# sikang/motion_primitive_library

Hardware: AMD Instinct MI355X
Metric: node-expansions/s (frontier x |U| pair evaluations per second) (higher is better)
Workload: dtype f64; 1 GPU; C4: 3D VoxelMapUtil 512^3, Control::ACC |U|=729 (9^3), 64k-node synthetic frontier; frontier=random, frontier_nodes=65536, frontier_nodes_per_gpu=65536, controls=729, dim=3, map_cells=134217728, device=AMD Radeon Graphics (gfx950:sramecc+:xnack-), compute_units=256, kernel=expand_lex_kernel

## Files before the change

### motion_primitive_library_amd/csrc/expand_lex_kernel.hip

```cpp
#include "mplx_internal.h"
#include "mplx_device_common.h"

namespace mplx {

using namespace dev;

constexpr int kLexWPB = 4;
constexpr int kLexBT = 64 * kLexWPB;
constexpr int kLexTabStride = 64;
constexpr int kLexUB8 = 8;

constexpr int kShUval = 0;
__host__ __device__ constexpr int lex_sh_tc(int TS) { return TS == 32 ? 768 : 384; }
__host__ __device__ constexpr int lex_sh_tt(int TS) { return lex_sh_tc(TS) + 64; }
__host__ __device__ constexpr int lex_ts(int ndp) { return ndp <= 8 ? 8 : (ndp <= 16 ? 16 : 32); }

__host__ __device__ constexpr int lex_fixed_bytes(int D, int K, int TS) {
  const int F = 4 * D + 2, KQ = K == 3 ? 4 : K;
  int w = (F * 8 + 15) & ~15;
  w += 128 + D * TS * 4 + D * TS * 4 * KQ + D * TS * 8 * (K - 1) + (K == 3 ? D * TS * 8 : 0) + D * TS + D * TS;
  w = (w + 15) & ~15;
  return (w + 128 + 7) & ~7;
}
__host__ __device__ constexpr int lex_tt_entries(int n_max) { return (n_max + 1) * (n_max + 2) / 2; }

template <int D, int K, int TS>
struct LexW {
  static constexpr int F = 4 * D + 2;
  static constexpr int KQ = K == 3 ? 4 : K;
  static constexpr int NODE = 0;
  static constexpr int MISC = (F * 8 + 15) & ~15;
  static constexpr int EFLAG = MISC + 128;
  static constexpr int EQ = EFLAG + D * TS * 4;
  static constexpr int EST = EQ + D * TS * 4 * KQ;
  static constexpr int UQ = EST + D * TS * 8 * (K - 1);
  static constexpr int VL = UQ + (K == 3 ? D * TS * 8 : 0);
  static constexpr int VLC = VL + D * TS;
  static constexpr int ROWMAP = (VLC + D * TS + 15) & ~15;
  static constexpr int HP = (ROWMAP + 128 + 7) & ~7;
  static_assert(HP == lex_fixed_bytes(D, K, TS), "LexLds sizes the workgroup's LDS from lex_fixed_bytes");
};
enum { LM_BASE = 0, LM_NODEQ = 4 };

struct LexLds {
  int tts, rowcap, o_wave0, w_drop, w_cell, w_box, wave_bytes, total;
  __host__ __device__ LexLds(int D, int K, int waves, int ndp, int nU, int n_max, int rmax, int boxcap) {
    tts = n_max + 1;
    rowcap = rmax * tts;
    o_wave0 = (lex_sh_tt(lex_ts(ndp)) + lex_tt_entries(n_max) * 8 + 15) & ~15;
    int w = lex_fixed_bytes(D, K, lex_ts(ndp));
    const int PN = (D == 3) ? ndp * ndp : ndp;
    w += PN * 8;
    w_drop = w;
    w += ((nU + 63) >> 6) * 8;
    w_cell = w;
    w += D * ndp * rowcap + 8;
    w = (w + 3) & ~3;
    w_box = w;
    w += boxcap * 4;
    wave_bytes = (w + 15) & ~15;
    total = o_wave0 + waves * wave_bytes;
  }
};

namespace {

template <typename T>
__device__ __forceinline__ void lex_st(T v, T *p) {
// ... 20 lines not shown
  x = op(x, __builtin_amdgcn_update_dpp(id, v, 0x111, 0xf, 0xf, false));
  x = op(x, __builtin_amdgcn_update_dpp(id, v, 0x112, 0xf, 0xf, false));
  x = op(x, __builtin_amdgcn_update_dpp(id, v, 0x113, 0xf, 0xf, false));
  x = op(x, __builtin_amdgcn_update_dpp(id, x, 0x114, 0xf, 0xe, false));
  x = op(x, __builtin_amdgcn_update_dpp(id, x, 0x118, 0xf, 0xc, false));
  return x;
}
__device__ __forceinline__ unsigned int row_reduce_or(unsigned int v) {
  int x = (int)v;
  x |= __builtin_amdgcn_update_dpp(0, (int)v, 0x111, 0xf, 0xf, false);
  x |= __builtin_amdgcn_update_dpp(0, (int)v, 0x112, 0xf, 0xf, false);
  x |= __builtin_amdgcn_update_dpp(0, (int)v, 0x113, 0xf, 0xf, false);
  x |= __builtin_amdgcn_update_dpp(0, x, 0x114, 0xf, 0xe, false);
  x |= __builtin_amdgcn_update_dpp(0, x, 0x118, 0xf, 0xc, false);
  return (unsigned int)x;
}

template <int K>
__device__ __forceinline__ void lex_fold_entry(uint64_t &h, const int *eq, int e) {
  if (K == 1) {
    fold(h, eq[e]);
  } else if (K == 2) {
    const int2 q = *(const int2 *)(eq + e * 2);
    fold(h, q.x);
    fold(h, q.y);
  } else {
    const int4 q = *(const int4 *)(eq + e * 4);
    fold(h, q.x);
    fold(h, q.y);
    fold(h, q.z);
  }
}

template <int D, int K, int TS>
__global__ __launch_bounds__(kLexBT) void expand_lex_kernel(const GridArgs A_kernarg) {
  extern __shared__ __align__(16) unsigned char smem[];
  typedef const GridArgs __attribute__((address_space(4))) *KernargPtr;
  KernargPtr Ak = (KernargPtr)__builtin_amdgcn_kernarg_segment_ptr();
  (void)A_kernarg;
#define A (*Ak)
  typedef LexW<D, K, TS> W;
  constexpr int F = W::F, KQ = W::KQ;
  constexpr int UB = (D == 3 && K == 3) ? 4 : kLexUB8;
  const int ndp = A.ndp, RM = A.rmax;
  const LexLds L(D, K, kLexWPB, ndp, A.nU, A.n_max, RM, A.boxcap);
  const int lane = threadIdx.x & 63;
  const int wv = __builtin_amdgcn_readfirstlane(threadIdx.x >> 6);
  const double *s_uval = (const double *)(smem + kShUval);
  constexpr int kShTc = lex_sh_tc(TS), kShTt = lex_sh_tt(TS);
  const unsigned char *s_tc = smem + kShTc;
  const double *s_tt = (const double *)(smem + kShTt);
  unsigned char *wb = smem + L.o_wave0 + wv * L.wave_bytes;
  double *s_node = (double *)(wb + W::NODE);
  int *s_misc = (int *)(wb + W::MISC);
  int *s_eflag = (int *)(wb + W::EFLAG);
  int *s_eq = (int *)(wb + W::EQ);
  double *s_est = (double *)(wb + W::EST);
  double *s_uq = (double *)(wb + W::UQ);
  unsigned char *s_vl = wb + W::VL;
  unsigned char *s_vlc = wb + W::VLC;
  unsigned short *s_rowmap = (unsigned short *)(wb + W::ROWMAP);
  uint64_t *s_drop = (uint64_t *)(wb + L.w_drop);
  uint64_t *s_hp = (uint64_t *)(wb + W::HP);
  unsigned char *s_cell = wb + L.w_cell;
  unsigned int *s_box = (unsigned int *)(wb + L.w_box);

  const int tts = L.tts, rowcap = L.rowcap;
  const int half = A.n_max + 2;
  const double T = A.dt;
  const int dims[3] = {A.dim0, A.dim1, A.dim2};
  const int nd[3] = {A.nd0, A.nd1, A.nd2};

  const int wave_id = (int)blockIdx.x * kLexWPB + wv;
  const int wave_stride = (int)gridDim.x * kLexWPB;
  const int NN = (int)A.n_nodes;
  const bool dyn = A.work != nullptr;
  const int ck = dyn ? A.work_chunk : 1;
  int dyn_beg = 0, dyn_len = 0, dyn_step = 1;
  unsigned int *ctr = nullptr;
  if (dyn) {
    if (blockIdx.x == 0 && threadIdx.x < kWorkCounters) A.work_zero[threadIdx.x * 32] = 0u;
    const int n_chunks = (NN + ck - 1) / ck, n_dyn = n_chunks > wave_stride ? n_chunks - wave_stride : 0;
    const int nc = gridDim.x < (unsigned)kWorkCounters ? (int)gridDim.x : kWorkCounters;
    const int cx = (int)(blockIdx.x % nc);
    const int base = n_dyn / nc, rem = n_dyn % nc;
    dyn_len = base + (cx < rem ? 1 : 0);
    if (A.work_blocked) { dyn_beg = wave_stride + cx * base + (cx < rem ? cx : rem); dyn_step = 1; }
    else { dyn_beg = wave_stride + cx; dyn_step = nc; }
    ctr = A.work + cx * 32;
  }
  auto claim = [&]() -> int {
    unsigned int v = 0;
    if (lane == 0) v = atomicAdd(ctr, 1u);
    const int j = __builtin_amdgcn_readfirstlane((int)v);
    return (j >= 0 && j < dyn_len) ? (dyn_beg + j * dyn_step) * ck : NN;
  };
  const int it0 = wave_id * ck;
  int chunk_end = it0 + ck < NN ? it0 + ck : NN;
  double nxt = 0.0;
  if (it0 < NN && lane < F) nxt = A.nodes[(int64_t)lane * A.node_stride + it0];
  int next_chunk = NN;
  if (dyn && it0 < NN) next_chunk = claim();

  {
// ... 61 lines not shown
    const int64_t node = it;
    lex_prio(0);
    lex_sync();
    if (lane < F) s_node[lane] = nxt;
    if (it_next < NN && lane < F) nxt = A.nodes[(int64_t)lane * A.node_stride + it_next];
    lex_sync();

    int flag[NR], rb_lo[NR], rb_hi[NR];
#pragma unroll
    for (int r = 0; r < NR; r++) {
    flag[r] = 0;
    rb_lo[r] = 0x7fffffff;
    rb_hi[r] = (int)0x80000000;
    const int ti_l = ti_r[r];
    if (ent_r[r]) {
      const int ax = ax_r[r];
      const double p = s_node[0 * D + ax];
      const double v = (K >= 2) ? s_node[1 * D + ax] : 0.0;
      const double a = (K >= 3) ? s_node[2 * D + ax] : 0.0;
      const double u = s_uval[ti_l];
      const double org = ax == 0 ? A.org0 : (ax == 1 ? A.org1 : A.org2);
      Ax<K> q;
      q.init(p, v, a, 0.0, u);
      const double mv = q.max_vel(T);
      bool valid = true;
      if (K >= 2 && A.v_max > 0) valid = valid && !(mv > A.v_max);
      if (K >= 3 && A.a_max > 0) valid = valid && !(q.max_acc(T) > A.a_max);
      int n = (int)ceil(div_by(mv * T, A.res, A.Rres));
      n = n < 5 ? 5 : (n > A.n_max ? A.n_max : n);
      const double np_ = q.template pos<true>(T);
      const double nv_ = q.template vel<true>(T);
      const double na_ = q.template acc<true>(T);
      if (K >= 3) s_uq[ti_l] = q.top_quotient();
      if (K >= 2) s_est[ti_l * (K - 1) + 0] = np_;
      if (K >= 3) s_est[ti_l * (K - 1) + 1] = nv_;
      s_eq[ti_l * KQ + 0] = quantise(np_, 0.01, A.R001);
      if (K >= 2) s_eq[ti_l * KQ + 1] = quantise(nv_, 0.1, A.R01);
      if (K >= 3) s_eq[ti_l * KQ + 2] = quantise(na_, 0.1, A.R01);
      flag[r] = (valid ? 1 : 0) | ((p == np_) ? 2 : 0) | (n << 8);
      if (A.sat != nullptr && valid) {
        double pmin = p < np_ ? p : np_, pmax = p < np_ ? np_ : p;
        if (K == 2 && u != 0) {
          const double ts = -v / u;
          if (ts > 0 && ts < T) {
            const double pe = q.template pos<false>(ts);
            pmin = pe < pmin ? pe : pmin;
            pmax = pe > pmax ? pe : pmax;
          }
        }
        if (K >= 3) { pmin = p - mv * T; pmax = p + mv * T; }
        rb_lo[r] = (int)floor(div_by(pmin - org, A.res, A.Rres)) - 1;
        rb_hi[r] = (int)floor(div_by(pmax - org, A.res, A.Rres)) + 1;
      }
      if (jv_l == 0) {
        const double qd = div_by(p - org, A.res, A.Rres);
        s_misc[LM_BASE + ax] = (qd - 0.5 > -0.5) ? (int)qd : -1;
      }
    } else if (LS == 16 && r == 0 && lane >= 48 && lane < 48 + 4 * D) {
      const int i = (lane - 48) >> 2, f = (lane - 48) & 3;
      if (f < K) {
        const double x = s_node[f * D + i];
        s_misc[LM_NODEQ + i * 4 + f] = f == 0 ? quantise(x, 0.01, A.R001) : quantise(x, 0.1, A.R01);
      }
    }
    if (ax_r[r] < D && jv_l < TS) s_eflag[ti_l] = flag[r];
    }
    if (LS == 32 && lane < 4 * D) {
      const int i = lane >> 2, f = lane & 3;
// ... 90 lines not shown
        bool ok = true;
#pragma unroll
        for (int i = 0; i < 2; i++) {
          e_lo[i] = rlo[i] - base_c[i] + half;
          const int hi = rhi[i] - base_c[i] + half;
          ok = ok && e_lo[i] >= 0 && hi <= 255;
          e_nb[i] = hi - e_lo[i] + 1;
        }
        eager = ok && e_nb[0] <= 32 && e_nb[1] <= 64 && e_nb[1] <= A.boxcap;
        if (eager) {
          const int xw = rlo[0], ay = rlo[1] + lane;
          const int vlo = xw < 0 ? -xw : 0;
          const int vhi = (dims[0] - xw) < 32 ? (dims[0] - xw) : 32;
          e_mask = (vhi >= 32 ? 0xffffffffu : ((1u << (vhi > 0 ? vhi : 0)) - 1u)) & ~((1u << vlo) - 1u);
          e_in = lane < e_nb[1] && vhi > vlo && ay >= 0 && ay < dims[1];
          const int64_t off = e_in ? (int64_t)ay * (int64_t)dims[0] + xw : 0;
          const int64_t wi = off >> 5;
          e_shf = (unsigned)(off & 31);
          const int64_t w0 = wi < 0 ? 0 : wi;
          const int64_t w1 = wi + 1 >= A.blk_words ? A.blk_words - 1 : wi + 1;
          e_a0 = A.blk[w0];
          e_a1 = A.blk[w1 < 0 ? 0 : w1];
        }
      }
      if (inside && lane < (1 << D)) {
        const int cx = (lane & 1) ? rhi[0] + 1 : rlo[0];
        const int cy = (lane & 2) ? rhi[1] + 1 : rlo[1];
        const int cz = (D == 3) ? ((lane & 4) ? rhi[2] + 1 : rlo[2]) : 1;
        const int64_t idx = cx + (int64_t)(dims[0] + 1) * (cy + (int64_t)(dims[1] + 1) * cz);
        sat_v = A.sat[idx];
      }
    }
    const double node_t = s_node[4 * D + 1];
    if (A.dbg & 1) nm = 0;
    asm volatile("" ::"v"(nxt));
    bool safe = false;
    if (A.sat != nullptr) {
      unsigned int term = (lane < (1 << D)) ? sat_v : 0u;
      if ((D - __popc((unsigned)lane & ((1u << D) - 1u))) & 1) term = 0u - term;
#pragma unroll
      for (int d = 1; d < (1 << D); d <<= 1) term += (unsigned int)__shfl_xor((int)term, d, 64);
      safe = sat_inside && __builtin_amdgcn_readfirstlane((int)term) == 0;
    }
    lex_sync();

    const int in1 = (D == 3) ? nv2 : 1, in0 = nv1 * in1;
    const float r_in0 = __builtin_amdgcn_rcpf((float)(in0 > 0 ? in0 : 1)), r_in1 = __builtin_amdgcn_rcpf((float)(in1 > 0 ? in1 : 1));
    int E = nA;

    lex_prio(1);
    for (int pass = 0; pass == 0 || nm != 0ull; pass++) {
      unsigned long long sub = 0;
      if (safe) {
        sub = ~0ull;
      } else {
        int used = 0;
        for (unsigned long long t = nm; t; t &= t - 1ull) {
          const int nn = __ffsll((long long)t) - 1;
          const int cn = (int)s_tc[nn];
          if (used + cn > rowcap && sub) break;
          sub |= 1ull << nn;
          used += cn;
        }
      }
      nm &= ~sub;
      lex_sync();
      {
        int off = 0;
// ... 66 lines not shown
      const bool fits = have_box && n_rows * WX <= A.boxcap;
      const int rot = (WX == 1) ? (lo[0] & 31) : 0;
      if (D == 2 && eager) {
        if (fits && pass == 0 && lane < nb[1]) {
          unsigned int val = e_in ? (__builtin_amdgcn_alignbit(e_a1, e_a0, e_shf) | ~e_mask) : 0xffffffffu;
          val = __builtin_amdgcn_alignbit(val, val, (32 - rot) & 31);
          s_box[lane] = val;
        }
      } else if (fits) {
        const float inv_ny = __builtin_amdgcn_rcpf((float)nb[1]);
        const int ax0 = base_c[0] + lo[0] - half;
        constexpr int SU = 4;
        const int ayb = base_c[1] + lo[1] - half, azb = (D == 3) ? base_c[2] + lo[2] - half : 0;
        for (int w = 0; w < WX; w++) {
          const int xw = ax0 + 32 * w;
          const int vlo = xw < 0 ? -xw : 0;
          const int vhi = (dims[0] - xw) < 32 ? (dims[0] - xw) : 32;
          const unsigned int mask = (vhi >= 32 ? 0xffffffffu : ((1u << (vhi > 0 ? vhi : 0)) - 1u)) & ~((1u << vlo) - 1u);
          for (int r0 = lane; r0 < n_rows; r0 += 64 * SU) {
            unsigned int a0[SU], a1[SU], shf[SU];
            bool in[SU];
#pragma unroll
            for (int u = 0; u < SU; u++) {
              const int r = r0 + 64 * u;
              const int rz = (D == 3) ? (int)(((float)r + 0.5f) * inv_ny) : 0;
              const int ry = r - rz * nb[1];
              const int ay = ayb + ry, az = azb + rz;
              in[u] = r < n_rows && vhi > vlo && ay >= 0 && ay < dims[1] && (D == 2 || (az >= 0 && az < dims[2]));
              const int64_t off = in[u] ? ((int64_t)az * dims[1] + ay) * (int64_t)dims[0] + xw : 0;
              const int64_t wi = off >> 5;
              shf[u] = (unsigned)(off & 31);
              const int64_t w0 = wi < 0 ? 0 : wi;
              const int64_t w1 = wi + 1 >= A.blk_words ? A.blk_words - 1 : wi + 1;
              a0[u] = (A.dbg & 8) ? 0u : A.blk[w0];
              a1[u] = (A.dbg & 8) ? 0u : A.blk[w1 < 0 ? 0 : w1];
            }
#pragma unroll
            for (int u = 0; u < SU; u++) {
              const int r = r0 + 64 * u;
              unsigned int val = in[u] ? (__builtin_amdgcn_alignbit(a1[u], a0[u], shf[u]) | ~mask) : 0xffffffffu;
              if (WX == 1) val = __builtin_amdgcn_alignbit(val, val, (32 - rot) & 31);
              if (r < n_rows) s_box[r * WX + w] = val;
            }
          }
        }
      }
      lex_sync();

      const int rowc = lo[1] + nb[1] * lo[2];
      int ndrop = 0;
      for (int x0 = 0; x0 < nA; x0 += 64) {
        const int x = x0 + lane;
        const bool act = x < nA;
        int j0 = 0, j1 = 0, j2 = 0;
        {
          const int xx = act ? x : 0;
          const int a_ = (int)(((float)xx + 0.5f) * r_in0);
          const int ra = xx - a_ * in0;
          int b_ = ra, c_ = 0;
          if (D == 3) {
            b_ = (int)(((float)ra + 0.5f) * r_in1);
            c_ = ra - b_ * in1;
          }
          j0 = s_vl[a_];
          j1 = s_vl[TS + b_];
          if (D == 3) j2 = s_vl[2 * TS + c_];
        }
        const int ci = (D == 3) ? (int)__umul24(__umul24(j0, nd[1]) + j1, nd[2]) + j2 : (int)__umul24(j0, nd[1]) + j1;
        const int en[3] = {j0, TS + j1, 2 * TS + j2};
        const int px = (D == 3) ? (int)__umul24(j0, ndp) + j1 : j0;
        int n, fl;
        {
          const int f0 = s_eflag[en[0]], f1 = s_eflag[en[1]];
          fl = f0 & f1 & 3;
          n = max(f0 >> 8, f1 >> 8);
          if (D == 3) {
            const int f2 = s_eflag[en[2]];
            fl &= f2;
            n = max(n, f2 >> 8);
          }
          if (fl & 2) n = 0;
        }
        uint64_t h = s_hp[px];
        lex_fold_entry<K>(h, s_eq, en[D - 1]);
        unsigned long long dm;
        if (pass == 0) {
          dm = __ballot(act && h == hcur);
          if (lane == 0) s_drop[x0 >> 6] = dm;
        } else {
          const uint64_t d_ = s_drop[x0 >> 6];
          dm = (unsigned long long)(unsigned int)__builtin_amdgcn_readfirstlane((int)(unsigned int)d_) |
               ((unsigned long long)(unsigned int)__builtin_amdgcn_readfirstlane((int)(unsigned int)(d_ >> 32)) << 32);
        }
        const bool dropped = (dm >> lane) & 1ull;
        const int e = x - ndrop - __popcll(dm & ((1ull << lane) - 1ull));
        ndrop += __popcll(dm);
        if (x0 + 64 >= nA) E = nA - ndrop;
        const bool emit = act && !dropped;
        const bool mine = emit && (n ? ((sub >> n) & 1ull) != 0ull : pass == 0);
        const int64_t idx = node * A.l_nstride + e;
        const bool past = !act && pass == 0 && A.l_pad;
        const bool pad16 = past && e < ((E + 15) & ~15);
        const bool pad32 = past && e < ((E + 31) & ~31);
        lex_prio(3);
        if ((mine || pad32) && !(A.dbg & 2)) {
          if (A.l_action) lex_st(mine ? ci : -1, &A.l_action[idx]);
          if (A.l_hash && (mine || pad16)) lex_st(h, &A.l_hash[idx]);
          if (A.l_state && (mine || pad16)) {
            double *o = A.l_state + idx;
            const int64_t ss = A.l_stride;
            const unsigned int zr = A.l_zrows;
#pragma unroll
            for (int i = 0; i < D; i++) {
              const double *st = s_est + en[i] * (K - 1);
              const double u = s_uval[en[i]];
              const double uK = 0.0 + u;
              const double top = (0.0 + u * T) + s_node[(K - 1) * D + i];
              lex_st((double)((K >= 2) ? st[0] : top), &o[(0 * D + i) * ss]);
              lex_st((double)((K >= 3) ? st[1] : (K == 2 ? top : uK)), &o[(1 * D + i) * ss]);
              if (K >= 2 || !((zr >> (2 * D + i)) & 1u)) lex_st((double)((K == 3) ? top : (K == 2 ? uK : 0.0)), &o[(2 * D + i) * ss]);
              if (K == 3 || !((zr >> (3 * D + i)) & 1u)) lex_st((double)((K == 3) ? uK : 0.0), &o[(3 * D + i) * ss]);
            }
            if (!((zr >> (4 * D)) & 1u)) lex_st(0.0, &o[(4 * D) * ss]);
            lex_st(node_t + A.dt, &o[(4 * D + 1) * ss]);
          }
          if ((A.post.heur || A.post.flags) && (mine || pad16)) {
            double pp[D], vv[D], aa[D];
#pragma unroll
            for (int i = 0; i < D; i++) {
              const double *st = s_est + en[i] * (K - 1);
              const double u = s_uval[en[i]];
              const double uK = 0.0 + u;
              const double top = (0.0 + u * T) + s_node[(K - 1) * D + i];
              pp[i] = (K >= 2) ? st[0] : top;
              vv[i] = (K >= 3) ? st[1] : (K == 2 ? top : uK);
              aa[i] = (K == 3) ? top : (K == 2 ? uK : 0.0);
            }
            double hv;
            unsigned int fv;
            MPLX_POST_GOAL(pg, A.post, D)
            post_eval<D>(pg, h, pp, vv, aa, 0.0, &hv, &fv);
            if (A.post.heur) lex_st(hv, &A.post.heur[idx]);
            if (A.post.flags && mine) A.post.flags[idx] = (uint8_t)fv;
          }
        }
        const bool smp = mine && n != 0;
        const int cntl = smp ? (int)s_tc[n] : 0;
        int fb = -1;
        {
          const int r = smp ? (int)s_rowmap[n] : 0;
          int ptr[3] = {0, 0, 0};
          ptr[0] = __umul24(j0, rowcap) + r;
          ptr[1] = __umul24(ndp + j1, rowcap) + r;
          if (D == 3) ptr[2] = __umul24(2 * ndp + j2, rowcap) + r;
          bool done = !smp || safe || (A.dbg & 32);
          if (fits) {
            if (WX == 1) {
              const unsigned int *bx = s_box - rowc;
              for (int k0 = 0; __ballot(!done) != 0ull; k0 += UB) {
                unsigned int m = 0;
#pragma unroll
                for (int q = 0; q < UB; q++) {
                  const int k = k0 + q;
                  const unsigned int ex = s_cell[ptr[0] + k];
                  const int ey = s_cell[ptr[1] + k];
                  const int ez = (D == 3) ? (int)s_cell[ptr[2] + k] : 0;
                  const unsigned int word = bx[(D == 3 ? (int)__umul24(nb[1], ez) : 0) + ey];
                  m |= __builtin_amdgcn_ubfe(word, ex, 1u) << q;
                }
                const int left = cntl - k0;
                if (left < UB) m &= (1u << (left > 0 ? left : 0)) - 1u;
                if (!done && m) { fb = k0 + __ffs((int)m) - 1; done = true; }
                if (left <= UB) done = true;
              }
            } else {
              for (int k0 = 0; __ballot(!done) != 0ull; k0 += UB) {
                unsigned int m = 0;
#pragma unroll
                for (int q = 0; q < UB; q++) {
                  const int k = k0 + q;
                  const int ex = s_cell[ptr[0] + k];
                  const int ey = s_cell[ptr[1] + k];
                  const int ez = (D == 3) ? (int)s_cell[ptr[2] + k] : 0;
                  const int dx = ex - lo[0];
                  const unsigned int word = s_box[__umul24((D == 3 ? (int)__umul24(nb[1], ez) : 0) + ey - rowc, WX) + (dx >> 5)];
                  m |= ((word >> (dx & 31)) & 1u) << q;
                }
                const int left = cntl - k0;
                if (left < UB) m &= (1u << (left > 0 ? left : 0)) - 1u;
                if (!done && m) { fb = k0 + __ffs((int)m) - 1; done = true; }
                if (left <= UB) done = true;
              }
            }
          } else {
            for (int k0 = 0; __ballot(!done) != 0ull; k0 += UB) {
              unsigned int wd[UB];
              int sh[UB];
#pragma unroll
              for (int q = 0; q < UB; q++) {
                int k = k0 + q;
                k = k < cntl ? k : (cntl > 0 ? cntl - 1 : 0);
                bool inside = !done;
                int64_t cell = 0, mul = 1;
#pragma unroll
                for (int i = 0; i < D; i++) {
                  const int c = base_c[i] + (done ? 0 : (int)s_cell[ptr[i] + k]) - half;
                  inside = inside && c >= 0 && c < dims[i];
                  cell += mul * c;
                  mul *= dims[i];
                }
                sh[q] = inside ? (int)(cell & 31) : -1;
                wd[q] = A.blk[inside ? (cell >> 5) : 0];
              }
#pragma unroll
              for (int q = 0; q < UB; q++) {
                if (!done && k0 + q < cntl && (sh[q] < 0 || ((wd[q] >> sh[q]) & 1u))) { fb = k0 + q; done = true; }
              }
              if (k0 + UB >= cntl) done = true;
            }
          }
        }
        if ((mine || pad32) && !(A.dbg & 4)) {
          const bool blocked = fb >= 0;
          double J = 0;
#pragma unroll
          for (int i = 0; i < D; i++) {
            const double u = s_uval[en[i]];
            J += u * u * T;
          }
          const double cost = blocked ? INFINITY : 0.0 + (J + A.w * A.dt);
          if (A.l_cost && (mine || pad16)) lex_st(cost, &A.l_cost[idx]);
          if (A.l_iters) lex_st(blocked ? fb + 1 : cntl, &A.l_iters[idx]);
        }
        lex_prio(1);
      }
      if (pass == 0 && lane == 0 && A.l_count) A.l_count[node] = E;
    }
  }
  if (A.done.flag != nullptr) {
    __threadfence_system();
    if (lane == 0) {
      const unsigned int waves = gridDim.x * (unsigned int)kLexWPB;
      if (__hip_atomic_fetch_add(A.done.count, 1u, __ATOMIC_ACQ_REL, __HIP_MEMORY_SCOPE_AGENT) == waves - 1u) {
        __hip_atomic_store(A.done.count, 0u, __ATOMIC_RELAXED, __HIP_MEMORY_SCOPE_AGENT);
        __hip_atomic_store(A.done.flag, A.done.seq, __ATOMIC_RELEASE, __HIP_MEMORY_SCOPE_SYSTEM);
      }
    }
  }
#undef A
}

template <int D, int K, int TS>
hipError_t lex_inst_attr() {
  static bool attr_set[64] = {};
  int dev = 0;
  if (hipGetDevice(&dev) != hipSuccess || dev < 0 || dev >= 64) dev = 63;
  if (!attr_set[dev] || dev == 63) {
    hipError_t e = hipFuncSetAttribute((const void *)expand_lex_kernel<D, K, TS>, hipFuncAttributeMaxDynamicSharedMemorySize, 160 * 1024);
    if (e != hipSuccess) return e;
    attr_set[dev] = true;
  }
  return hipSuccess;
}

template <int D, int K, int TS>
hipError_t launch_lex_ts(const GridArgs &a, hipStream_t stream) {
  if (a.n_nodes == 0) return hipSuccess;
  const int64_t n_wg = (a.n_nodes + kLexWPB - 1) / kLexWPB;
  const int64_t blocks = n_wg < (int64_t)a.grid_limit ? n_wg : (int64_t)a.grid_limit;
  const size_t lds = lex_lds_bytes(D, K, a.ndp, a.nU, a.n_max, a.rmax, a.boxcap);
  if (hipError_t e = lex_inst_attr<D, K, TS>()) return e;
  hipLaunchKernelGGL((expand_lex_kernel<D, K, TS>), dim3((unsigned)blocks), dim3(kLexBT), lds, stream, a);
  return hipGetLastError();
}
template <int D, int K>
hipError_t launch_lex_inst(const GridArgs &a, hipStream_t stream) {
  return a.ndp <= 8 ? launch_lex_ts<D, K, 8>(a, stream) : (a.ndp <= 16 ? launch_lex_ts<D, K, 16>(a, stream) : launch_lex_ts<D, K, 32>(a, stream));
}

template <int D, int K, int TS>
int lex_resident_ts(size_t lds) {
  if (lex_inst_attr<D, K, TS>() != hipSuccess) return 0;
  int nb = 0;
  if (hipOccupancyMaxActiveBlocksPerMultiprocessor(&nb, (const void *)expand_lex_kernel<D, K, TS>, kLexBT, lds) != hipSuccess) {
    (void)hipGetLastError();
    return 0;
  }
  return nb;
}
template <int D, int K>
int lex_resident_inst(size_t lds, int ndp) {
  return ndp <= 8 ? lex_resident_ts<D, K, 8>(lds) : (ndp <= 16 ? lex_resident_ts<D, K, 16>(lds) : lex_resident_ts<D, K, 32>(lds));
}

}

size_t lex_lds_bytes(int dim, int order, int ndp, int nU, int n_max, int rmax, int boxcap) {
  return (size_t)LexLds(dim, order, kLexWPB, ndp, nU, n_max, rmax, boxcap).total;
}
int lex_waves_per_block() { return kLexWPB; }

bool lex_covers(int dim, int control) {
  return (dim == 2 || dim == 3) && (control == 0x01 || control == 0x03 || control == 0x07);
}

hipError_t launch_expand_lex(int dim, int control, const GridArgs &a, hipStream_t s) {
  if (dim == 2) {
    switch (control) {
      case 0x01: return launch_lex_inst<2, 1>(a, s);
      case 0x03: return launch_lex_inst<2, 2>(a, s);
      case 0x07: return launch_lex_inst<2, 3>(a, s);
    }
  } else if (dim == 3) {
    switch (control) {
      case 0x01: return launch_lex_inst<3, 1>(a, s);
      case 0x03: return launch_lex_inst<3, 2>(a, s);
      case 0x07: return launch_lex_inst<3, 3>(a, s);
    }
  }
  return hipErrorInvalidValue;
}
// ... 20 lines not shown
```

### motion_primitive_library_amd/csrc/lists_route.cpp

```cpp
#include "mplx_ctx.h"

#include <cmath>
#include <cstdio>
#include <cstdlib>

namespace mplx_detail {


template <class Args>
static void set_env(const mplx_ctx *c, Args *a) {
  a->region = c->has_region ? (const uint32_t *)c->region_bits.p : nullptr;
  a->dim0 = c->mdim[0]; a->dim1 = c->mdim[1]; a->dim2 = c->mdim[2];
  a->org0 = c->origin[0]; a->org1 = c->origin[1]; a->org2 = c->origin[2];
  a->res = c->res;
  a->dt = c->prm.dt; a->w = c->prm.w;
  a->v_max = c->prm.v_max; a->a_max = c->prm.a_max; a->j_max = c->prm.j_max;
}

template <class Args>
static void set_tables(const mplx_ctx *c, Args *a) {
  a->ttab = (const double *)c->tables.p;
  a->tcnt = (const unsigned char *)c->tables.p + kTcntOffset;
  a->Rres = c->recips[0]; a->R001 = c->recips[1]; a->R01 = c->recips[2];
}
// ... 226 lines not shown
}

static int grid_work(mplx_ctx *c, mplx::GridArgs *a) {
  a->work = nullptr;
  a->work_zero = nullptr;
  a->work_chunk = 1;
  const int64_t wpb = mplx::grid_waves_per_block();
  const int64_t n_wg = (a->n_nodes + wpb - 1) / wpb;
  const int64_t W = (n_wg < (int64_t)a->grid_limit ? n_wg : (int64_t)a->grid_limit) * wpb;
  if (c->tune.grid_static || a->n_nodes <= W) return MPLX_OK;
  const size_t set_bytes = (size_t)mplx::kWorkCounters * 128;
  if (!c->work_counter.p) {
    if (int rc = ensure(c, c->work_counter, 2 * set_bytes)) return rc;
    HIP_TRY(c, hipMemsetAsync(c->work_counter.p, 0, 2 * set_bytes, c->stream));
    c->work_parity = 0;
  }
  a->work = (unsigned int *)((char *)c->work_counter.p + (c->work_parity ? set_bytes : 0));
  a->work_zero = (unsigned int *)((char *)c->work_counter.p + (c->work_parity ? 0 : set_bytes));
  int64_t per_wave = a->n_nodes / W, ck = per_wave / 16;
  if (ck < 1) ck = 1;
  if (ck > 8) ck = 8;
  if (c->tune.grid_chunk > 0) ck = c->tune.grid_chunk;
  a->work_chunk = (int32_t)ck;
  a->work_blocked = c->tune.grid_blocked ? 1 : 0;
  return MPLX_OK;
}

int launch_grid(mplx_ctx *c, mplx::GridArgs *a) {
  if (int rc = grid_work(c, a)) return rc;
  const hipError_t e = a->lex ? mplx::launch_expand_lex(c->dim, c->prm.control, *a, c->stream)
                              : mplx::launch_expand_grid(c->dim, c->prm.control, *a, c->stream);
  c->last_grid_lex = a->lex != 0;
  c->last_grid_pair = false;
  if (e != hipSuccess) {
    if (a->work) {
      (void)hipStreamSynchronize(c->stream);
      release(c->work_counter);
    }
    return fail(c, MPLX_ERR_HIP, "expand_grid_kernel launch failed: %s", hipGetErrorString(e));
  }
  if (a->work) c->work_parity ^= 1;
  return MPLX_OK;
}

static int launch_pair(mplx_ctx *c, const PairPlan &pp, const mplx::GridArgs &a) {
  mplx::GridArgs b = a;
  b.rmax = pp.rmax;
  b.grid_limit = pp.grid;
  b.work = nullptr;
  b.work_zero = nullptr;
  const hipError_t e = mplx::launch_expand_pair(c->dim, c->prm.control, b, c->stream);
  if (e != hipSuccess) return fail(c, MPLX_ERR_HIP, "expand_pair_kernel launch failed: %s", hipGetErrorString(e));
  c->last_grid_lex = false;
  c->last_grid_pair = true;
  return MPLX_OK;
}

static int prescreen(mplx_ctx *c, const GridPlan &gp, mplx::GridArgs *a) {
  const bool yaw = (c->prm.control & 0x10) != 0;
  const int64_t n_nodes = a->n_nodes;
  const int64_t ps_min = c->tune.prescreen_min > 0 ? c->tune.prescreen_min : (int64_t)4 * gp.grid * mplx::grid_waves_per_block();
  if (!(yaw && gp.order >= 2 && c->prm.yaw_max > 0 && c->tune.prescreen_min >= 0 && n_nodes >= ps_min && n_nodes < 0x7fffffffLL))
    return MPLX_OK;
  if (int rc = ensure(c, c->live_list, (size_t)n_nodes * 4)) return rc;
  if (!c->live_ctr.p) {
    if (int rc = ensure(c, c->live_ctr, 256)) return rc;
// ... 34 lines not shown
  HIP_TRY(c, mplx::launch_build_blocked_bits((const int8_t *)(c->has_pot ? c->pot.p : c->map.p),
                                             c->has_region ? (const uint32_t *)c->region_bits.p : nullptr, c->n_cells,
                                             c->has_pot ? 1 : 0, (uint32_t *)c->blk.p, c->stream));
  c->sat_ok = false;
  if (int rc = rebuild_sat(c)) return rc;
  c->blk_ok = true;
  return MPLX_OK;
}

int ensure_tables(mplx_ctx *c) {
  if (c->tables_ok && c->tab_dt == c->prm.dt && c->tab_res == c->res) return MPLX_OK;
  const size_t bytes = kTcntOffset + 64 + 64;
  if (int rc = ensure(c, c->tables, bytes)) return rc;
  double *ttab = (double *)c->tables.p;
  unsigned char *tcnt = (unsigned char *)c->tables.p + kTcntOffset;
  double *rec = (double *)((unsigned char *)c->tables.p + kTcntOffset + 64);
  HIP_TRY(c, hipMemsetAsync(c->tables.p, 0, bytes, c->stream));
  HIP_TRY(c, mplx::launch_make_tables(c->prm.dt, c->res, ttab, tcnt, rec, c->stream));
  HIP_TRY(c, hipMemcpyAsync(c->recips, rec, 3 * sizeof(double), hipMemcpyDeviceToHost, c->stream));
  HIP_TRY(c, hipStreamSynchronize(c->stream));
  c->tab_dt = c->prm.dt;
  c->tab_res = c->res;
  c->tables_ok = true;
  return MPLX_OK;
}

static uint32_t const_zero_rows(int dim, int control) {
  const int order = control_order(control);
  uint32_t m = 0;
  for (int b = order + 1; b <= 3; b++)
    for (int i = 0; i < dim; i++) m |= 1u << (b * dim + i);
  if (!(control & 0x10)) m |= 1u << (4 * dim);
  return m;
}

static mplx::GridArgs grid_args(mplx_ctx *c, const GridPlan &gp, const double *d_nodes, int64_t n_nodes, int64_t node_stride,
                                const mplx_succ_lists *o, uint32_t skip) {
  mplx::GridArgs a{};
  set_env(c, &a);
  set_tables(c, &a);
  set_lists(c, o, &a);
  a.blk = (const uint32_t *)c->blk.p;
  a.blk_words = (c->n_cells + 31) >> 5;
  a.pot = c->has_pot ? (const int8_t *)c->pot.p : nullptr;
  a.pot_w = c->prm.potential_weight;
  a.grad_w = c->has_pot ? c->prm.gradient_weight : 0.0;
  const bool yaw = (c->prm.control & 0x10) != 0;
  a.sat = (c->sat_ok && gp.order <= 3 && !(yaw && c->prm.wyaw > 0) && !c->tune.no_sat && gp.use_sat)
              ? (const uint32_t *)c->sat.p : nullptr;
  a.gather = gp.gather ? 1 : 0;
  a.yaw_max = c->prm.yaw_max; a.wyaw = c->prm.wyaw; a.ndy = yaw ? c->u_nd[3] : 0;
  a.uvals = (const double *)c->uvals.p + (c->u_wide ? 4 * 16 : 0);
  a.uval_stride = c->u_wide ? 32 : 16;
  a.uidx = (const uint32_t *)c->uidx.p;
  a.nd0 = c->u_nd[0]; a.nd1 = c->u_nd[1]; a.nd2 = c->u_nd[2];
  a.ndp = gp.ndp;
  a.ulex = gp.ulex;
  a.nU = c->nU;
  a.nodes = d_nodes; a.n_nodes = n_nodes; a.node_stride = node_stride;
  a.n_max = gp.n_max; a.rmax = gp.rmax; a.boxcap = gp.boxcap; a.grid_limit = gp.grid;
  a.lex = gp.lex ? 1 : 0;
  a.dbg = c->tune.dbg;
  a.l_pad = line_pad(c, a.l_nstride);
  a.l_zrows = skip;
  a.post = post_of(c, o);
  return a;
}

static int lists_grid(mplx_ctx *c, const GridPlan &gp, const double *d_nodes, int64_t n_nodes, int64_t node_stride,
                      const mplx_succ_lists *o, uint32_t skip) {
  if (int rc = ensure_tables(c)) return rc;
  if (int rc = ensure_blocked_bits(c)) return rc;
  if (c->sat_stale && n_nodes >= 4096)
    if (int rc = rebuild_sat(c)) return rc;
  mplx::GridArgs a = grid_args(c, gp, d_nodes, n_nodes, node_stride, o, skip);
  if (int rc = yaw_slot(c, &a.yaw)) return rc;
  if (int rc = prescreen(c, gp, &a)) return rc;
  arm_done(c, &a.done);
  const PairPlan pp = plan_pair(c, gp, a);
  if (int rc = pp.ok ? launch_pair(c, pp, a) : launch_grid(c, &a)) return rc;
  c->done_armed = a.done.flag != nullptr;
  if (a.yaw.amb) {
    mplx_ctx::YawPending p;
    p.kind = 0;
    p.g = a;
    p.g.live = nullptr;
    p.g.live_n = nullptr;
    p.g.done = {};
    c->yaw_pending.push_back(p);
  }
  c->last_route = MPLX_ROUTE_GRID;
  return MPLX_OK;
}

static int lists_tile(mplx_ctx *c, const TilePlan &tp, const double *d_nodes, int64_t n_nodes, int64_t node_stride,
                      const mplx_succ_lists *o) {
  if (int rc = ensure_tables(c)) return rc;
  mplx::TileArgs a = tile_args(c, tp, d_nodes, n_nodes, node_stride, o);
// ... 146 lines not shown
```

Measured before the change: 109.8 billion pairs/s.

## Add specialised hot lex kernel variants with compile-time store and collision paths

Adds template variants of the lex expansion kernel (edges-only and with state rows), selected on the host when the output configuration matches the common case. These variants drop run-time debug and null-pointer checks, pick the collision-check path (safe, LDS single-word, LDS multi-word, direct) at compile time, and write outputs with inline-asm nontemporal global stores using 32-bit offsets. Per-control terms (the top state component and u*u*T) are precomputed once per control into LDS, so the per-edge loops read them instead of recomputing. In exchange, per-wave LDS grows, up to five copies of the loop body raise code size, and occupancy now takes the minimum across all variants.

```diff
diff --git a/motion_primitive_library_amd/csrc/expand_lex_kernel.hip b/motion_primitive_library_amd/csrc/expand_lex_kernel.hip
--- a/motion_primitive_library_amd/csrc/expand_lex_kernel.hip
+++ b/motion_primitive_library_amd/csrc/expand_lex_kernel.hip
@@ -1,5 +1,7 @@
 #include "mplx_internal.h"
 #include "mplx_device_common.h"
+
+#include <type_traits>
 
 namespace mplx {
 
@@ -18,7 +20,7 @@
 __host__ __device__ constexpr int lex_fixed_bytes(int D, int K, int TS) {
   const int F = 4 * D + 2, KQ = K == 3 ? 4 : K;
   int w = (F * 8 + 15) & ~15;
-  w += 128 + D * TS * 4 + D * TS * 4 * KQ + D * TS * 8 * (K - 1) + (K == 3 ? D * TS * 8 : 0) + D * TS + D * TS;
+  w += 128 + D * TS * 4 + D * TS * 4 * KQ + D * TS * 8 * (K + 1) + (K == 3 ? D * TS * 8 : 0) + D * TS + D * TS;
   w = (w + 15) & ~15;
   return (w + 128 + 7) & ~7;
 }
@@ -32,8 +34,9 @@
   static constexpr int MISC = (F * 8 + 15) & ~15;
   static constexpr int EFLAG = MISC + 128;
   static constexpr int EQ = EFLAG + D * TS * 4;
+  static constexpr int ES = K + 1;
   static constexpr int EST = EQ + D * TS * 4 * KQ;
-  static constexpr int UQ = EST + D * TS * 8 * (K - 1);
+  static constexpr int UQ = EST + D * TS * 8 * ES;
   static constexpr int VL = UQ + (K == 3 ? D * TS * 8 : 0);
   static constexpr int VLC = VL + D * TS;
   static constexpr int ROWMAP = (VLC + D * TS + 15) & ~15;
@@ -120,15 +123,27 @@
   }
 }
 
-template <int D, int K, int TS>
+enum { LV_GEN = 0, LV_STATE = 1, LV_EDGES = 2 };
+enum { SM_GEN = 0, SM_SAFE, SM_LDS1, SM_LDSN, SM_DIRECT };
+
+template <typename T>
+__device__ __forceinline__ void lex_st_at(T v, T *base, unsigned int off) {
+  if constexpr (sizeof(T) == 8)
+    asm volatile("s_nop 4\n\tglobal_store_dwordx2 %0, %1, %2 sc1 nt" ::"v"(off), "v"(v), "s"(base) : "memory");
+  else
+    asm volatile("s_nop 4\n\tglobal_store_dword %0, %1, %2 sc1 nt" ::"v"(off), "v"(v), "s"(base) : "memory");
+}
+
+template <int D, int K, int TS, int V>
 __global__ __launch_bounds__(kLexBT) void expand_lex_kernel(const GridArgs A_kernarg) {
   extern __shared__ __align__(16) unsigned char smem[];
+  constexpr bool HOT = V != LV_GEN, ST = V == LV_STATE;
   typedef const GridArgs __attribute__((address_space(4))) *KernargPtr;
   KernargPtr Ak = (KernargPtr)__builtin_amdgcn_kernarg_segment_ptr();
   (void)A_kernarg;
 #define A (*Ak)
   typedef LexW<D, K, TS> W;
-  constexpr int F = W::F, KQ = W::KQ;
+  constexpr int F = W::F, KQ = W::KQ, ES = W::ES;
   constexpr int UB = (D == 3 && K == 3) ? 4 : kLexUB8;
   const int ndp = A.ndp, RM = A.rmax;
   const LexLds L(D, K, kLexWPB, ndp, A.nU, A.n_max, RM, A.boxcap);
@@ -158,6 +173,13 @@
   const double T = A.dt;
   const int dims[3] = {A.dim0, A.dim1, A.dim2};
   const int nd[3] = {A.nd0, A.nd1, A.nd2};
+  int32_t *const h_action = HOT ? A.l_action : nullptr;
+  uint64_t *const h_hash = HOT ? A.l_hash : nullptr;
+  double *const h_cost = HOT ? A.l_cost : nullptr;
+  double *const h_state = ST ? A.l_state : nullptr;
+  const int64_t h_ss = ST ? A.l_stride : 0, h_ns = HOT ? A.l_nstride : 0;
+  const bool h_pad = HOT && A.l_pad;
+  const double h_dt = HOT ? A.dt : 0.0, h_wdt = HOT ? A.w * A.dt : 0.0;
 
   const int wave_id = (int)blockIdx.x * kLexWPB + wv;
   const int wave_stride = (int)gridDim.x * kLexWPB;
@@ -285,8 +307,10 @@
       const double nv_ = q.template vel<true>(T);
       const double na_ = q.template acc<true>(T);
       if (K >= 3) s_uq[ti_l] = q.top_quotient();
-      if (K >= 2) s_est[ti_l * (K - 1) + 0] = np_;
-      if (K >= 3) s_est[ti_l * (K - 1) + 1] = nv_;
+      if (K >= 2) s_est[ti_l * ES + 0] = np_;
+      if (K >= 3) s_est[ti_l * ES + 1] = nv_;
+      s_est[ti_l * ES + (K - 1)] = (0.0 + u * T) + (K == 1 ? p : (K == 2 ? v : a));
+      s_est[ti_l * ES + K] = u * u * T;
       s_eq[ti_l * KQ + 0] = quantise(np_, 0.01, A.R001);
       if (K >= 2) s_eq[ti_l * KQ + 1] = quantise(nv_, 0.1, A.R01);
       if (K >= 3) s_eq[ti_l * KQ + 2] = quantise(na_, 0.1, A.R01);
@@ -443,8 +467,14 @@
       }
     }
     const double node_t = s_node[4 * D + 1];
-    if (A.dbg & 1) nm = 0;
+    if (!HOT && (A.dbg & 1)) nm = 0;
     asm volatile("" ::"v"(nxt));
+    if (D == 2) asm volatile("" ::"v"(e_a0), "v"(e_a1));
+    const double t_next = node_t + (HOT ? h_dt : 0.0);
+    int32_t *const nb_action = HOT ? h_action + node * h_ns : nullptr;
+    uint64_t *const nb_hash = HOT ? h_hash + node * h_ns : nullptr;
+    double *const nb_cost = HOT ? h_cost + node * h_ns : nullptr;
+    double *const nb_state = ST ? h_state + node * h_ns : nullptr;
     bool safe = false;
     if (A.sat != nullptr) {
       unsigned int term = (lane < (1 << D)) ? sat_v : 0u;
@@ -577,8 +607,8 @@
               shf[u] = (unsigned)(off & 31);
               const int64_t w0 = wi < 0 ? 0 : wi;
               const int64_t w1 = wi + 1 >= A.blk_words ? A.blk_words - 1 : wi + 1;
-              a0[u] = (A.dbg & 8) ? 0u : A.blk[w0];
-              a1[u] = (A.dbg & 8) ? 0u : A.blk[w1 < 0 ? 0 : w1];
+              a0[u] = (!HOT && (A.dbg & 8)) ? 0u : A.blk[w0];
+              a1[u] = (!HOT && (A.dbg & 8)) ? 0u : A.blk[w1 < 0 ? 0 : w1];
             }
 #pragma unroll
             for (int u = 0; u < SU; u++) {
@@ -587,6 +617,8 @@
               if (WX == 1) val = __builtin_amdgcn_alignbit(val, val, (32 - rot) & 31);
               if (r < n_rows) s_box[r * WX + w] = val;
             }
+#pragma unroll
+            for (int u = 0; u < SU; u++) asm volatile("" ::"v"(a0[u]), "v"(a1[u]));
           }
         }
       }
@@ -594,7 +626,9 @@
 
       const int rowc = lo[1] + nb[1] * lo[2];
       int ndrop = 0;
-      for (int x0 = 0; x0 < nA; x0 += 64) {
+      auto step = [&](auto sm_c, const int x0) {
+        constexpr int SM = decltype(sm_c)::value;
+        static_assert(HOT ? SM != SM_GEN : SM == SM_GEN, "the general body tests at run time what the hot loops are built for");
         const int x = x0 + lane;
         const bool act = x < nA;
         int j0 = 0, j1 = 0, j2 = 0;
@@ -643,12 +677,36 @@
         if (x0 + 64 >= nA) E = nA - ndrop;
         const bool emit = act && !dropped;
         const bool mine = emit && (n ? ((sub >> n) & 1ull) != 0ull : pass == 0);
-        const int64_t idx = node * A.l_nstride + e;
-        const bool past = !act && pass == 0 && A.l_pad;
+        const int64_t idx = HOT ? 0 : node * A.l_nstride + e;
+        const bool past = !act && pass == 0 && (HOT ? h_pad : A.l_pad != 0);
         const bool pad16 = past && e < ((E + 15) & ~15);
         const bool pad32 = past && e < ((E + 31) & ~31);
+        const unsigned int o8 = (unsigned int)e * 8u;
         lex_prio(3);
-        if ((mine || pad32) && !(A.dbg & 2)) {
+        if constexpr (HOT) {
+          if (mine || pad32) {
+            lex_st_at(mine ? ci : -1, nb_action, (unsigned int)e * 4u);
+            if (mine || pad16) {
+              lex_st_at(h, nb_hash, o8);
+              if constexpr (ST) {
+                int64_t ss = h_ss;
+                asm volatile("" : "+s"(ss));
+                double *row = nb_state;
+#pragma unroll
+                for (int i = 0; i < D; i++, row += ss) {
+                  const double *st = s_est + en[i] * ES;
+                  const double uK = 0.0 + s_uval[en[i]];
+                  const double top = st[K - 1];
+                  lex_st_at((double)((K >= 2) ? st[0] : top), row, o8);
+                  lex_st_at((double)((K >= 3) ? st[1] : (K == 2 ? top : uK)), row + D * ss, o8);
+                  if (K >= 2) lex_st_at((double)((K == 3) ? top : uK), row + 2 * D * ss, o8);
+                  if (K == 3) lex_st_at(uK, row + 3 * D * ss, o8);
+                }
+                lex_st_at(t_next, row + (3 * D + 1) * ss, o8);
+              }
+            }
+          }
+        } else if ((mine || pad32) && !(A.dbg & 2)) {
           if (A.l_action) lex_st(mine ? ci : -1, &A.l_action[idx]);
           if (A.l_hash && (mine || pad16)) lex_st(h, &A.l_hash[idx]);
           if (A.l_state && (mine || pad16)) {
@@ -657,10 +715,9 @@
             const unsigned int zr = A.l_zrows;
 #pragma unroll
             for (int i = 0; i < D; i++) {
-              const double *st = s_est + en[i] * (K - 1);
-              const double u = s_uval[en[i]];
-              const double uK = 0.0 + u;
-              const double top = (0.0 + u * T) + s_node[(K - 1) * D + i];
+              const double *st = s_est + en[i] * ES;
+              const double uK = 0.0 + s_uval[en[i]];
+              const double top = st[K - 1];
               lex_st((double)((K >= 2) ? st[0] : top), &o[(0 * D + i) * ss]);
               lex_st((double)((K >= 3) ? st[1] : (K == 2 ? top : uK)), &o[(1 * D + i) * ss]);
               if (K >= 2 || !((zr >> (2 * D + i)) & 1u)) lex_st((double)((K == 3) ? top : (K == 2 ? uK : 0.0)), &o[(2 * D + i) * ss]);
@@ -673,10 +730,9 @@
             double pp[D], vv[D], aa[D];
 #pragma unroll
             for (int i = 0; i < D; i++) {
-              const double *st = s_est + en[i] * (K - 1);
-              const double u = s_uval[en[i]];
-              const double uK = 0.0 + u;
-              const double top = (0.0 + u * T) + s_node[(K - 1) * D + i];
+              const double *st = s_est + en[i] * ES;
+              const double uK = 0.0 + s_uval[en[i]];
+              const double top = st[K - 1];
               pp[i] = (K >= 2) ? st[0] : top;
               vv[i] = (K >= 3) ? st[1] : (K == 2 ? top : uK);
               aa[i] = (K == 3) ? top : (K == 2 ? uK : 0.0);
@@ -692,15 +748,16 @@
         const bool smp = mine && n != 0;
         const int cntl = smp ? (int)s_tc[n] : 0;
         int fb = -1;
-        {
+        if constexpr (SM != SM_SAFE) {
           const int r = smp ? (int)s_rowmap[n] : 0;
           int ptr[3] = {0, 0, 0};
           ptr[0] = __umul24(j0, rowcap) + r;
           ptr[1] = __umul24(ndp + j1, rowcap) + r;
           if (D == 3) ptr[2] = __umul24(2 * ndp + j2, rowcap) + r;
-          bool done = !smp || safe || (A.dbg & 32);
-          if (fits) {
-            if (WX == 1) {
+          bool done = !smp;
+          if constexpr (SM == SM_GEN) done = done || safe || (A.dbg & 32);
+          if (SM == SM_GEN ? fits : SM != SM_DIRECT) {
+            if (SM == SM_GEN ? WX == 1 : SM == SM_LDS1) {
               const unsigned int *bx = s_box - rowc;
               for (int k0 = 0; __ballot(!done) != 0ull; k0 += UB) {
                 unsigned int m = 0;
@@ -761,23 +818,41 @@
               for (int q = 0; q < UB; q++) {
                 if (!done && k0 + q < cntl && (sh[q] < 0 || ((wd[q] >> sh[q]) & 1u))) { fb = k0 + q; done = true; }
               }
+              if constexpr (HOT) {
+#pragma unroll
+                for (int q = 0; q < UB; q++) asm volatile("" ::"v"(wd[q]));
+              }
               if (k0 + UB >= cntl) done = true;
             }
           }
         }
-        if ((mine || pad32) && !(A.dbg & 4)) {
+        bool costs = mine || pad32;
+        if constexpr (!HOT) costs = costs && !(A.dbg & 4);
+        if (costs) {
           const bool blocked = fb >= 0;
           double J = 0;
 #pragma unroll
-          for (int i = 0; i < D; i++) {
-            const double u = s_uval[en[i]];
-            J += u * u * T;
+          for (int i = 0; i < D; i++) J += s_est[en[i] * ES + K];
+          if constexpr (HOT) {
+            if (mine || pad16) lex_st_at(blocked ? (double)INFINITY : 0.0 + (J + h_wdt), nb_cost, o8);
+          } else {
+            const double cost = blocked ? INFINITY : 0.0 + (J + A.w * A.dt);
+            if (A.l_cost && (mine || pad16)) lex_st(cost, &A.l_cost[idx]);
+            if (A.l_iters) lex_st(blocked ? fb + 1 : cntl, &A.l_iters[idx]);
           }
-          const double cost = blocked ? INFINITY : 0.0 + (J + A.w * A.dt);
-          if (A.l_cost && (mine || pad16)) lex_st(cost, &A.l_cost[idx]);
-          if (A.l_iters) lex_st(blocked ? fb + 1 : cntl, &A.l_iters[idx]);
         }
         lex_prio(1);
+      };
+      if constexpr (!HOT) {
+        for (int x0 = 0; x0 < nA; x0 += 64) step(std::integral_constant<int, SM_GEN>(), x0);
+      } else if (safe) {
+        for (int x0 = 0; x0 < nA; x0 += 64) step(std::integral_constant<int, SM_SAFE>(), x0);
+      } else if (fits && WX == 1) {
+        for (int x0 = 0; x0 < nA; x0 += 64) step(std::integral_constant<int, SM_LDS1>(), x0);
+      } else if (fits) {
+        for (int x0 = 0; x0 < nA; x0 += 64) step(std::integral_constant<int, SM_LDSN>(), x0);
+      } else {
+        for (int x0 = 0; x0 < nA; x0 += 64) step(std::integral_constant<int, SM_DIRECT>(), x0);
       }
       if (pass == 0 && lane == 0 && A.l_count) A.l_count[node] = E;
     }
@@ -795,43 +870,53 @@
 #undef A
 }
 
-template <int D, int K, int TS>
+template <int D, int K, int TS, int V>
 hipError_t lex_inst_attr() {
   static bool attr_set[64] = {};
   int dev = 0;
   if (hipGetDevice(&dev) != hipSuccess || dev < 0 || dev >= 64) dev = 63;
   if (!attr_set[dev] || dev == 63) {
-    hipError_t e = hipFuncSetAttribute((const void *)expand_lex_kernel<D, K, TS>, hipFuncAttributeMaxDynamicSharedMemorySize, 160 * 1024);
+    hipError_t e = hipFuncSetAttribute((const void *)expand_lex_kernel<D, K, TS, V>, hipFuncAttributeMaxDynamicSharedMemorySize, 160 * 1024);
     if (e != hipSuccess) return e;
     attr_set[dev] = true;
   }
   return hipSuccess;
 }
 
-template <int D, int K, int TS>
-hipError_t launch_lex_ts(const GridArgs &a, hipStream_t stream) {
+template <int D, int K, int TS, int V>
+hipError_t launch_lex_v(const GridArgs &a, hipStream_t stream) {
   if (a.n_nodes == 0) return hipSuccess;
   const int64_t n_wg = (a.n_nodes + kLexWPB - 1) / kLexWPB;
   const int64_t blocks = n_wg < (int64_t)a.grid_limit ? n_wg : (int64_t)a.grid_limit;
   const size_t lds = lex_lds_bytes(D, K, a.ndp, a.nU, a.n_max, a.rmax, a.boxcap);
-  if (hipError_t e = lex_inst_attr<D, K, TS>()) return e;
-  hipLaunchKernelGGL((expand_lex_kernel<D, K, TS>), dim3((unsigned)blocks), dim3(kLexBT), lds, stream, a);
+  if (hipError_t e = lex_inst_attr<D, K, TS, V>()) return e;
+  hipLaunchKernelGGL((expand_lex_kernel<D, K, TS, V>), dim3((unsigned)blocks), dim3(kLexBT), lds, stream, a);
   return hipGetLastError();
+}
+template <int D, int K, int TS>
+hipError_t launch_lex_ts(const GridArgs &a, hipStream_t stream) {
+  if (a.lex != 2) return launch_lex_v<D, K, TS, LV_GEN>(a, stream);
+  return a.l_state ? launch_lex_v<D, K, TS, LV_STATE>(a, stream) : launch_lex_v<D, K, TS, LV_EDGES>(a, stream);
 }
 template <int D, int K>
 hipError_t launch_lex_inst(const GridArgs &a, hipStream_t stream) {
   return a.ndp <= 8 ? launch_lex_ts<D, K, 8>(a, stream) : (a.ndp <= 16 ? launch_lex_ts<D, K, 16>(a, stream) : launch_lex_ts<D, K, 32>(a, stream));
 }
 
+template <int D, int K, int TS, int V>
+int lex_resident_v(size_t lds) {
+  if (lex_inst_attr<D, K, TS, V>() != hipSuccess) return 0;
+  int nb = 0;
+  if (hipOccupancyMaxActiveBlocksPerMultiprocessor(&nb, (const void *)expand_lex_kernel<D, K, TS, V>, kLexBT, lds) != hipSuccess) {
+    (void)hipGetLastError();
+    return 0;
+  }
+  return nb;
+}
 template <int D, int K, int TS>
 int lex_resident_ts(size_t lds) {
-  if (lex_inst_attr<D, K, TS>() != hipSuccess) return 0;
-  int nb = 0;
-  if (hipOccupancyMaxActiveBlocksPerMultiprocessor(&nb, (const void *)expand_lex_kernel<D, K, TS>, kLexBT, lds) != hipSuccess) {
-    (void)hipGetLastError();
-    return 0;
-  }
-  return nb;
+  const int g = lex_resident_v<D, K, TS, LV_GEN>(lds), s = lex_resident_v<D, K, TS, LV_STATE>(lds), e = lex_resident_v<D, K, TS, LV_EDGES>(lds);
+  return g < s ? (g < e ? g : e) : (s < e ? s : e);
 }
 template <int D, int K>
 int lex_resident_inst(size_t lds, int ndp) {
diff --git a/motion_primitive_library_amd/csrc/lists_route.cpp b/motion_primitive_library_amd/csrc/lists_route.cpp
--- a/motion_primitive_library_amd/csrc/lists_route.cpp
+++ b/motion_primitive_library_amd/csrc/lists_route.cpp
@@ -282,6 +282,9 @@
                               : mplx::launch_expand_grid(c->dim, c->prm.control, *a, c->stream);
   c->last_grid_lex = a->lex != 0;
   c->last_grid_pair = false;
+  if (a->lex && getenv("MPLX_GRID_VERBOSE"))
+    fprintf(stderr, "mplx: lex launch of %lld nodes: %s\n", (long long)a->n_nodes,
+            a->lex != 2 ? "general body" : (a->l_state ? "hot variant, state rows" : "hot variant, edges only"));
   if (e != hipSuccess) {
     if (a->work) {
       (void)hipStreamSynchronize(c->stream);
@@ -382,6 +385,15 @@
     for (int i = 0; i < dim; i++) m |= 1u << (b * dim + i);
   if (!(control & 0x10)) m |= 1u << (4 * dim);
   return m;
+}
+
+static bool lex_hot_scope(const mplx_ctx *c, const mplx::GridArgs &a) {
+  const char *e = getenv("MPLX_LEX_HOT");
+  if (e && atoi(e) == 0) return false;
+  if (!a.l_count || !a.l_action || !a.l_cost || !a.l_hash || a.l_iters || a.post.heur || a.post.flags || a.dbg) return false;
+  if (a.l_nstride >= (1 << 28)) return false;
+  const uint32_t zero_rows = const_zero_rows(c->dim, c->prm.control);
+  return !a.l_state || (a.l_zrows & zero_rows) == zero_rows;
 }
 
 static mplx::GridArgs grid_args(mplx_ctx *c, const GridPlan &gp, const double *d_nodes, int64_t n_nodes, int64_t node_stride,
@@ -414,6 +426,7 @@
   a.l_pad = line_pad(c, a.l_nstride);
   a.l_zrows = skip;
   a.post = post_of(c, o);
+  if (a.lex && lex_hot_scope(c, a)) a.lex = 2;
   return a;
 }
 
```

Result: faster. 111.7 billion pairs/s (median of 6 runs) (+1.7%).
